# thanard/me-trpo

Hardware: AMD Instinct MI355X
Metric: imagined env-steps/sec (KxBxH) over the full TRPO iteration (higher is better)
Workload: dtype f32

## Files before the change

### me-trpo_amd/csrc/policy_mfma.hip

```cpp
#include <type_traits>
#include "device_common.h"
#include "cg_device.h"

typedef float f32x4 __attribute__((ext_vector_type(4)));
typedef float f32x2 __attribute__((ext_vector_type(2)));
#define PKFMA(a, b, c) __builtin_elementwise_fma((a), (b), (c))
#define MFMA16(a, b, c) __builtin_amdgcn_mfma_f32_16x16x4f32((a), (b), (c), 0, 0, 0)
#define PART_EXTRA 3
#ifndef POL_SKIP
#define POL_SKIP 0
#endif
#ifndef POL_SPLIT_R
#define POL_SPLIT_R 13
#endif
#ifndef POL_SPLIT_R_FVP
#define POL_SPLIT_R_FVP 7
#endif
#ifndef NWAVES
#define NWAVES 8
#endif
constexpr int cdiv_(int a, int b) { return (a + b - 1) / b; }
static_assert(POL_SPLIT_R == 0 || (NWAVES == 8 && (POL_SPLIT_R & 1) == 1 && POL_SPLIT_R >= 3 && (POL_SPLIT_R_FVP & 1) == 1 && POL_SPLIT_R_FVP >= 3), "the uneven deal pairs wave w with wave w + 4");
#ifdef POL_TIMING
__device__ unsigned long long g_pol_phase[16][8];
#define PT_MARK(i) { if (MODE_ == OP_FVPC && blockIdx.x == 0 && lane == 0) g_pol_phase[wave][i] = __builtin_readcyclecounter(); }
extern "C" int32_t metrpo_debug_pol_phases(unsigned long long* out) { return hipMemcpyFromSymbol(out, HIP_SYMBOL(g_pol_phase), sizeof(unsigned long long) * 128) == hipSuccess ? 0 : -1; }
#else
#define PT_MARK(i)
#endif


__device__ __forceinline__ void wave_sync_lds() {
    __builtin_amdgcn_fence(__ATOMIC_SEQ_CST, "wavefront");
    __builtin_amdgcn_wave_barrier();
}
__device__ __forceinline__ float xsum_q(float v) {
    typedef unsigned u32x2_ __attribute__((ext_vector_type(2)));
    const u32x2_ a = __builtin_amdgcn_permlane16_swap(__float_as_uint(v), __float_as_uint(v), false, false);
    const float s = __uint_as_float(a[0]) + __uint_as_float(a[1]);
    const u32x2_ b = __builtin_amdgcn_permlane32_swap(__float_as_uint(s), __float_as_uint(s), false, false);
    return __uint_as_float(b[0]) + __uint_as_float(b[1]);
}
template <int CTRL> __device__ __forceinline__ float dpp_add(float v) {
    return v + __int_as_float(__builtin_amdgcn_update_dpp(0, __float_as_int(v), CTRL, 0xF, 0xF, true));
}
__device__ __forceinline__ float xsum_c(float v) {
    v = dpp_add<0xB1>(v); v = dpp_add<0x4E>(v); v = dpp_add<0x141>(v); v = dpp_add<0x140>(v);
    return v;
}


template <int NS, int NA, int PH>
struct PolImg {
    static constexpr int NS_KS = cdiv_(NS, 4), HB = cdiv_(PH, 16), KK = HB * 4;
    static constexpr int O_W0F = 0, O_W1F = O_W0F + NS_KS * 64 * HB, O_V0F = O_W1F + KK * 64 * HB, O_V1F = O_V0F + NS_KS * 64 * HB,
                         O_W2B = O_V1F + KK * 64 * HB, O_W1B = O_W2B + 4 * 64 * HB, O_W2F = O_W1B + KK * 64 * HB,
                         O_V2F = O_W2F + KK * 64, TOTAL = O_V2F + KK * 64;
};


template <int NS, int NA, int PH, int MODE_>
__device__ __forceinline__ void pol_body(const PolK& k, const float* __restrict__ theta, const float* __restrict__ v, float* __restrict__ partials) {
    using I = PolImg<NS, NA, PH>;
    constexpr bool CACHED = (MODE_ == OP_FVPC), VPG = (MODE_ == OP_VPG), PPOKL = (MODE_ == OP_PPOKL), PPO = (MODE_ == OP_PPO) || PPOKL;
    constexpr int MODE = CACHED ? OP_FVP : (VPG || PPO) ? OP_GRAD : MODE_;
    constexpr int NS_KS = I::NS_KS, NSI = cdiv_(NS, 16), HB = I::HB, KK = I::KK;
    constexpr int pW0 = 0, pb0 = NS * PH, pW1 = pb0 + PH, pb1 = pW1 + PH * PH, pW2 = pb1 + PH, pb2 = pW2 + PH * NA,
                  pLS = pb2 + NA, P = pLS + NA, ROW = P + PART_EXTRA;
    constexpr int TS = 20, TILE = 16 * TS;
    constexpr int WTL = (3 * HB + (NA <= 2 ? 0 : 1)) * TILE;
    extern __shared__ __attribute__((aligned(16))) float lds[];
    const int tid = threadIdx.x, lane = tid & 63, wave = __builtin_amdgcn_readfirstlane(tid >> 6);
    const int c = lane & 15, q = lane >> 4;
    if (MODE_ == OP_LOSSKL && k.skip != nullptr && k.skip[0] >= 0.0) return;
    float* IMG = lds;
    float* TL = lds + I::TOTAL + wave * WTL;
    PT_MARK(0)
    const long long ntiles = (k.N + 15) / 16;
    const f32x4* __restrict__ hc = (const f32x4*)k.hcache;
    const bool ols_const = !VPG && (MODE != OP_FVP) && k.ls_stride == 0 && k.old_ls != nullptr;
    struct TileIn {
        float xB[NS_KS]; float xTs[4][NSI]; float ols[4], omu[4], act[4], adv; f32x4 gmv; int vld, nrem; f32x4 h[2 * HB];
    };
    auto fetch = [&](long long tile_, TileIn& in) {
        const long long tile = (tile_ < ntiles) ? tile_ : ntiles - 1;
        const long long n0 = tile * 16;
        const int nrem = (int)((k.N - n0 < 16) ? k.N - n0 : 16);
        in.nrem = nrem;
        const int cl = (c < nrem) ? c : nrem - 1;
        const float* __restrict__ ob = k.obs + n0 * NS;
#pragma unroll
        for (int s = 0; s < NS_KS; ++s) { const int f = 4 * s + q; in.xB[s] = ob[cl * NS + ((f < NS) ? f : NS - 1)]; }
        if (MODE != OP_LOSSKL) {
#pragma unroll
            for (int s = 0; s < 4; ++s) {
                const int sl = 4 * q + s, slc = (sl < nrem) ? sl : nrem - 1;
#pragma unroll
                for (int ci = 0; ci < NSI; ++ci) { const int f = 16 * ci + c; in.xTs[s][ci] = ob[slc * NS + ((f < NS) ? f : NS - 1)]; }
            }
        }
        in.vld = (k.valid == nullptr) ? 1 : (int)k.valid[n0 + cl];
        if (MODE != OP_FVP) {
            const long long nl = n0 + cl;
            if (MODE == OP_GRAD && k.gm != nullptr) {
#pragma unroll
                for (int r = 0; r < 4; ++r) { const int d = 4 * q + r; in.gmv[r] = k.gm[nl * NA + ((d < NA) ? d : NA - 1)]; }
            } else {
#pragma unroll
                for (int r = 0; r < 4; ++r) {
                    const int d = 4 * q + r, dc = (d < NA) ? d : NA - 1;
                    if (VPG) { in.act[r] = k.act[nl * NA + dc]; continue; }
                    in.ols[r] = ols_const ? 0.f : k.old_ls[(size_t)nl * k.ls_stride + dc]; in.omu[r] = k.old_mean[nl * NA + dc]; in.act[r] = k.act[nl * NA + dc];
                }
                in.adv = k.adv[nl];
            }
        }
        if (CACHED) {
            const f32x4* __restrict__ hb_ = hc + tile * (2 * HB) * 64;
#pragma unroll
            for (int j = 0; j < 2 * HB; ++j) in.h[j] = hb_[j * 64 + lane];
        }
    };
    auto mask_tile = [&](TileIn& in) {
#pragma unroll
        for (int s = 0; s < NS_KS; ++s) if (4 * s + 3 >= NS && 4 * s + q >= NS) in.xB[s] = 0.f;
        if (in.nrem == 16) return;
        const bool inr = c < in.nrem;
#pragma unroll
        for (int s = 0; s < NS_KS; ++s) if (!inr) in.xB[s] = 0.f;
#pragma unroll
        for (int s = 0; s < 4; ++s)
#pragma unroll
            for (int ci = 0; ci < NSI; ++ci) if (4 * q + s >= in.nrem) in.xTs[s][ci] = 0.f;
        if (!inr) { in.vld = 0; in.adv = 0.f; }
#pragma unroll
        for (int r = 0; r < 4; ++r) if (!inr) { in.ols[r] = 0.f; in.omu[r] = 0.f; in.act[r] = 0.f; in.gmv[r] = 0.f; }
    };
    TileIn nxt;

#define FRAG2(off, row, cb) IMG[(off) + ((row) * 64 + lane) * HB + (cb)]
#define FRAG1(off, row) IMG[(off) + (row) * 64 + lane]
    f32x4 b0f[HB], b1f[HB], b2f;
#pragma unroll
    for (int cb = 0; cb < HB; ++cb)
#pragma unroll
        for (int r = 0; r < 4; ++r) { const int u = 16 * cb + 4 * q + r; b0f[cb][r] = (u < PH) ? theta[pb0 + u] : 0.f; b1f[cb][r] = (u < PH) ? theta[pb1 + u] : 0.f; }
#pragma unroll
    for (int r = 0; r < 4; ++r) b2f[r] = (4 * q + r < NA) ? theta[pb2 + 4 * q + r] : 0.f;
    float ls[4], inv_std[4];
#pragma unroll
    for (int r = 0; r < 4; ++r) { ls[r] = (4 * q + r < NA) ? fmaxf(theta[pLS + 4 * q + r], LOG_MIN_STD) : 0.f; inv_std[r] = expf(-ls[r]); }
    float fisher_w[4];
#pragma unroll
    for (int r = 0; r < 4; ++r) fisher_w[r] = 1.0f / (expf(2.f * ls[r]) + 0.5f * KL_EPS);
    float ols_c[4] = {0.f, 0.f, 0.f, 0.f}, eo_c[4] = {1.f, 1.f, 1.f, 1.f}, os2_c[4] = {1.f, 1.f, 1.f, 1.f};
    if (ols_const) {
#pragma unroll
        for (int r = 0; r < 4; ++r)
            if (4 * q + r < NA) { ols_c[r] = k.old_ls[4 * q + r]; eo_c[r] = expf(-ols_c[r]); os2_c[r] = expf(2.f * ols_c[r]); }
    }
    constexpr bool kl_open = PPOKL;
    const float kl_w = PPOKL ? k.kl_beta * k.inv_n : 0.f, kl_d = PPOKL ? (float)k.kl_delta : 0.f;
    f32x4 vb0f[HB], vb1f[HB], vb2f;
    if (MODE == OP_FVP) {
#pragma unroll
        for (int cb = 0; cb < HB; ++cb)
#pragma unroll
            for (int r = 0; r < 4; ++r) { const int u = 16 * cb + 4 * q + r; vb0f[cb][r] = (u < PH) ? v[pb0 + u] : 0.f; vb1f[cb][r] = (u < PH) ? v[pb1 + u] : 0.f; }
#pragma unroll
        for (int r = 0; r < 4; ++r) vb2f[r] = (4 * q + r < NA) ? v[pb2 + 4 * q + r] : 0.f;
    }
    constexpr bool L2V = (NA <= 2);
    constexpr int NAV = L2V ? NA : 1;
    float w2l[HB][4][NAV], v2l[HB][4][NAV], gw2l[HB][4][NAV], b2l[NAV], vb2l[NAV], fisher_d[NAV];
    if (L2V) {
#pragma unroll
        for (int cb = 0; cb < HB; ++cb)
#pragma unroll
            for (int r = 0; r < 4; ++r)
#pragma unroll
                for (int d = 0; d < NAV; ++d) {
                    const int u = 16 * cb + 4 * q + r;
                    w2l[cb][r][d] = (u < PH) ? theta[pW2 + u * NA + d] : 0.f;
                    v2l[cb][r][d] = (MODE == OP_FVP && u < PH) ? v[pW2 + u * NA + d] : 0.f;
                    gw2l[cb][r][d] = 0.f;
                }
#pragma unroll
        for (int d = 0; d < NAV; ++d) {
            b2l[d] = theta[pb2 + d]; vb2l[d] = (MODE == OP_FVP) ? v[pb2 + d] : 0.f;
            fisher_d[d] = 1.0f / (expf(2.f * fmaxf(theta[pLS + d], LOG_MIN_STD)) + 0.5f * KL_EPS);
        }
    }
    constexpr int SPL = POL_SPLIT_R ? ((MODE == OP_GRAD || MODE_ == OP_FVP) ? POL_SPLIT_R : POL_SPLIT_R_FVP) : 0;
    const long long first_tile = SPL ? (long long)blockIdx.x * 4 + (wave & 3) + ((wave < 4) ? 0 : 1) * (long long)gridDim.x * 4 : (long long)blockIdx.x * NWAVES + wave;
    if (CACHED && k.imgval != nullptr) {
        static_assert(I::TOTAL % 4 == 0, "image tables are multiples of 64 floats");
        constexpr int NQ = I::TOTAL / 4, NIT = cdiv_(NQ, NWAVES * 64);
        float4 w4[NIT];
#pragma unroll
        for (int it = 0; it < NIT; ++it) { const int i = it * NWAVES * 64 + tid; w4[it] = (i < NQ) ? ((const float4*)k.imgval)[i] : make_float4(0.f, 0.f, 0.f, 0.f); }
        asm volatile("" ::: "memory");
        fetch(first_tile, nxt);
#pragma unroll
        for (int it = 0; it < NIT; ++it) { const int i = it * NWAVES * 64 + tid; if (i < NQ) ((float4*)IMG)[i] = w4[it]; }
    } else {
        constexpr int IMG_U = 8;
#pragma unroll
        for (int i0 = 0; i0 < I::TOTAL; i0 += NWAVES * 64 * IMG_U) {
            int m[IMG_U]; float w[IMG_U];
#pragma unroll
            for (int u = 0; u < IMG_U; ++u) { const int i = i0 + u * NWAVES * 64 + tid; m[u] = (i < I::TOTAL) ? k.img_map[i] : -1; }
#pragma unroll
            for (int u = 0; u < IMG_U; ++u) {
                const int i = i0 + u * NWAVES * 64 + tid;
                bool use = m[u] >= 0;
                if (MODE != OP_FVP && (m[u] & 0x40000000)) use = false;
                if (MODE == OP_LOSSKL && i >= I::O_W2B && i < I::O_W2F) use = false;
                if (CACHED && i < I::O_W1F) use = false;
                w[u] = 0.f;
                if (use) w[u] = (m[u] & 0x40000000) ? v[m[u] & 0x3FFFFFFF] : theta[m[u]];
            }
            if (i0 + NWAVES * 64 * IMG_U >= I::TOTAL) { asm volatile("" ::: "memory"); fetch(first_tile, nxt); asm volatile("" ::: "memory"); }
#pragma unroll
            for (int u = 0; u < IMG_U; ++u) { const int i = i0 + u * NWAVES * 64 + tid; if (i < I::TOTAL) IMG[i] = w[u]; }
        }
    }
    __syncthreads();
    if (MODE_ == OP_GRAD && k.imgval != nullptr && blockIdx.x == 0) {
        for (int i = tid; i < I::TOTAL; i += NWAVES * 64) k.imgval[i] = IMG[i];
    }
    PT_MARK(1)

    const f32x4 Z4 = {0.f, 0.f, 0.f, 0.f};
    f32x4 gW0[NSI][HB], gW1[HB][HB], gW2[HB], gb0[HB], gb1[HB], gb2 = Z4;
#pragma unroll
    for (int a = 0; a < HB; ++a) {
        gW2[a] = Z4; gb0[a] = Z4; gb1[a] = Z4;
#pragma unroll
        for (int b = 0; b < HB; ++b) gW1[a][b] = Z4;
#pragma unroll
        for (int b = 0; b < NSI; ++b) gW0[b][a] = Z4;
    }
    float dls[4] = {0.f, 0.f, 0.f, 0.f};
    float acc0 = 0.f, acc1 = 0.f, accw = 0.f;

    __builtin_amdgcn_s_waitcnt(0x0F70);
    PT_MARK(2)
    const long long sp_base = SPL ? (long long)blockIdx.x * 4 + (wave & 3) : (long long)blockIdx.x * NWAVES + wave, sp_stride = (long long)gridDim.x * (SPL ? 4 : NWAVES);
    auto sp_next = [&](long long m) -> long long {
        if constexpr (SPL == 0) return m + 1;
        else { const int ph = (int)(m % SPL); return (wave < 4) ? ((ph == SPL - 1) ? m + 1 : m + 2) : ((ph == SPL - 2) ? m + 3 : m + 2); }
    };
    for (long long m = (SPL && wave >= 4) ? 1 : 0, tile = sp_base + m * sp_stride; tile < ntiles; m = sp_next(m), tile = sp_base + m * sp_stride) {
        const long long n0 = tile * 16, n = n0 + c;
        const bool inr = n < k.N;
        TileIn in = nxt;
        fetch(sp_base + sp_next(m) * sp_stride, nxt);
        asm volatile("" ::: "memory");
        mask_tile(in);
        const bool ok = inr && in.vld != 0;
        const float (&xB)[NS_KS] = in.xB;
        const float (&xTs)[4][NSI] = in.xTs;
        const int wpos = c;
        float* T_H0 = TL, *T_H1 = TL + HB * TILE, *T_D1 = TL + 2 * HB * TILE, *T_UM = TL + 3 * HB * TILE;
        f32x4 h0[HB], h1[HB], t0[HB], t1[HB];
        constexpr bool H0C = CACHED;
        if (CACHED) {
#pragma unroll
            for (int cb = 0; cb < HB; ++cb) { if (H0C) h0[cb] = in.h[cb]; h1[cb] = in.h[HB + cb]; }
        }
#pragma unroll
        for (int cb = 0; cb < HB; ++cb) { if (!H0C) h0[cb] = b0f[cb]; if (MODE == OP_FVP) t0[cb] = vb0f[cb]; }
#pragma unroll
        for (int s = 0; s < NS_KS; ++s)
#pragma unroll
            for (int cb = 0; cb < HB; ++cb) {
                if (!H0C) h0[cb] = MFMA16(FRAG2(I::O_W0F, s, cb), xB[s], h0[cb]);
                if (MODE == OP_FVP) t0[cb] = MFMA16(FRAG2(I::O_V0F, s, cb), xB[s], t0[cb]);
            }
#pragma unroll
        for (int cb = 0; cb < HB; ++cb) {
            if (!CACHED) h1[cb] = b1f[cb];
            if (MODE == OP_FVP) t1[cb] = vb1f[cb];
            if (!H0C) {
#pragma unroll
                for (int r = 0; r < 4; ++r) h0[cb][r] = tanh_fast(h0[cb][r]);
            }
        }
#pragma unroll
        for (int kk = 0; kk < KK; ++kk)
#pragma unroll
            for (int cb = 0; cb < HB; ++cb) {
                if (!CACHED) h1[cb] = MFMA16(FRAG2(I::O_W1F, kk, cb), h0[kk >> 2][kk & 3], h1[cb]);
                if (MODE == OP_FVP) { if (POL_SKIP & 4) t1[cb][0] += h0[kk >> 2][kk & 3]; else t1[cb] = MFMA16(FRAG2(I::O_V1F, kk, cb), h0[kk >> 2][kk & 3], t1[cb]); }
            }
        if (MODE != OP_LOSSKL) {
#pragma unroll
            for (int cb = 0; cb < HB; ++cb)
#pragma unroll
                for (int r = 0; r < ((POL_SKIP & 8) ? 0 : 4); ++r) T_H0[cb * TILE + (4 * q + r) * TS + wpos] = h0[cb][r];
        }
        if (MODE == OP_FVP) {
#pragma unroll
            for (int cb = 0; cb < HB; ++cb)
#pragma unroll
                for (int r = 0; r < 4; ++r) t0[cb][r] *= fmaf(-h0[cb][r], h0[cb][r], 1.f);
#pragma unroll
            for (int kk = 0; kk < KK; ++kk)
#pragma unroll
                for (int cb = 0; cb < HB; ++cb) { if (POL_SKIP & 4) t1[cb][1] += t0[kk >> 2][kk & 3]; else t1[cb] = MFMA16(FRAG2(I::O_W1F, kk, cb), t0[kk >> 2][kk & 3], t1[cb]); }
        }
        if (!CACHED) {
#pragma unroll
            for (int cb = 0; cb < HB; ++cb)
#pragma unroll
                for (int r = 0; r < 4; ++r) h1[cb][r] = tanh_fast(h1[cb][r]);
        }
        if (MODE != OP_LOSSKL) {
#pragma unroll
            for (int cb = 0; cb < HB; ++cb)
#pragma unroll
                for (int r = 0; r < (((POL_SKIP & 8) || NA <= 2) ? 0 : 4); ++r) T_H1[cb * TILE + (4 * q + r) * TS + wpos] = h1[cb][r];
        }
        if (MODE == OP_GRAD && k.hcache != nullptr) {
            f32x4* hw = (f32x4*)k.hcache + (size_t)tile * (2 * HB) * 64 + lane;
#pragma unroll
            for (int cb = 0; cb < HB; ++cb) { hw[cb * 64] = h0[cb]; hw[(HB + cb) * 64] = h1[cb]; }
        }

        f32x4 um = Z4;
        float ual[NAV];
#pragma unroll
        for (int d = 0; d < NAV; ++d) ual[d] = 0.f;
        if (MODE == OP_GRAD && k.gm != nullptr) {
#pragma unroll
            for (int r = 0; r < 4; ++r) um[r] = (ok && 4 * q + r < NA) ? in.gmv[r] : 0.f;
        } else if (MODE != OP_FVP) {
            f32x4 mu = Z4;
            if (L2V) {
#pragma unroll
                for (int d = 0; d < NAV; ++d) {
                    float a = 0.f;
#pragma unroll
                    for (int cb = 0; cb < HB; ++cb)
#pragma unroll
                        for (int r = 0; r < 4; ++r) a = fmaf(w2l[cb][r][d], h1[cb][r], a);
                    a = xsum_q(a) + b2l[d];
                    if (q == 0) mu[d] = a;
                }
            } else {
                f32x4 m0 = b2f, m1 = Z4;
#pragma unroll
                for (int kk = 0; kk < KK; kk += 2) {
                    m0 = MFMA16(FRAG1(I::O_W2F, kk), h1[kk >> 2][kk & 3], m0);
                    m1 = MFMA16(FRAG1(I::O_W2F, kk + 1), h1[(kk + 1) >> 2][(kk + 1) & 3], m1);
                }
                mu = m0 + m1;
            }
            float llr = 0.f, kl = 0.f, zz[4] = {0.f, 0.f, 0.f, 0.f};
            float kmu[4] = {0.f, 0.f, 0.f, 0.f}, kls[4] = {0.f, 0.f, 0.f, 0.f};
#pragma unroll
            for (int r = 0; r < 4; ++r) {
                const int d = 4 * q + r;
                if (VPG && d < NA && ok) {
                    const float z = (in.act[r] - mu[r]) * inv_std[r];
                    llr -= ls[r] + 0.5f * z * z;
                    zz[r] = z;
                } else if (d < NA && ok) {
                    const float omu = in.omu[r], a = in.act[r];
                    float ols, eo, os2 = 0.f;
                    if (ols_const) { ols = ols_c[r]; eo = eo_c[r]; os2 = os2_c[r]; }
                    else {
                        ols = in.ols[r];
                        asm volatile("" : "+v"(ols));
                        eo = expf(-ols);
                        if (MODE == OP_LOSSKL || (PPOKL && kl_open)) os2 = expf(2.f * ols);
                    }
                    const float z = (a - mu[r]) * inv_std[r], zo = (a - omu) * eo;
                    llr += (ols - ls[r]) + 0.5f * (zo * zo - z * z);
                    zz[r] = z;
                    if (MODE == OP_LOSSKL) {
                        const float s2 = expf(2.f * ls[r]), dm = omu - mu[r];
                        kl += (dm * dm + os2 - s2) / (2.f * s2 + KL_EPS) + ls[r] - ols;
                    }
                    if constexpr (PPOKL) { if (kl_open) kl += ppo_kl_dim(mu[r], omu, ls[r], ols, os2, inv_std[r], &kmu[r], &kls[r]); }
                }
            }
            llr = xsum_q(llr);
            float la, surr;
            if constexpr (PPO) { la = ppo_gate(expf(llr), in.adv, k.clip_lo, k.clip_hi, &surr); if (!ok) { la = 0.f; surr = 0.f; } }
            else { la = ok ? (VPG ? in.adv : expf(llr) * in.adv) : 0.f; surr = VPG ? (llr - NA * HALF_LOG_2PI) * la : la; }
            if (q == 0) acc0 -= surr * k.inv_n;
            if (MODE == OP_LOSSKL) { acc1 += kl * k.inv_n; continue; }
            const float w = -la * k.inv_n;
#pragma unroll
            for (int r = 0; r < 4; ++r) {
                um[r] = w * zz[r] * inv_std[r];
                if (4 * q + r < NA) dls[r] += w * (zz[r] * zz[r] - 1.f);
            }
            if constexpr (PPOKL) {
                if (kl_open) {
                    acc0 += kl_w * kl;
                    if (q == 0 && ok) acc0 -= kl_w * kl_d;
#pragma unroll
                    for (int r = 0; r < 4; ++r) { um[r] += kl_w * kmu[r]; if (4 * q + r < NA) dls[r] += kl_w * kls[r]; }
                }
            }
        } else {
            f32x4 m0 = vb2f, m1 = Z4;
            if (!L2V) {
#pragma unroll
                for (int kk = 0; kk < KK; ++kk) m1 = MFMA16(FRAG1(I::O_V2F, kk), h1[kk >> 2][kk & 3], m1);
            }
#pragma unroll
            for (int cb = 0; cb < HB; ++cb)
#pragma unroll
                for (int r = 0; r < 4; ++r) t1[cb][r] *= fmaf(-h1[cb][r], h1[cb][r], 1.f);
            if (L2V) {
                m0 = Z4;
                float av[NAV];
                if constexpr (NAV == 2) {
                    f32x2 a2 = {0.f, 0.f};
#pragma unroll
                    for (int cb = 0; cb < HB; ++cb)
#pragma unroll
                        for (int r = 0; r < 4; ++r)
                            a2 = PKFMA((f32x2{w2l[cb][r][0], w2l[cb][r][1]}), (f32x2{t1[cb][r], t1[cb][r]}),
                                       PKFMA((f32x2{v2l[cb][r][0], v2l[cb][r][1]}), (f32x2{h1[cb][r], h1[cb][r]}), a2));
                    av[0] = a2[0]; av[1] = a2[1];
                } else {
#pragma unroll
                    for (int d = 0; d < NAV; ++d) {
                        av[d] = 0.f;
#pragma unroll
                        for (int cb = 0; cb < HB; ++cb)
#pragma unroll
                            for (int r = 0; r < 4; ++r) av[d] = fmaf(w2l[cb][r][d], t1[cb][r], fmaf(v2l[cb][r][d], h1[cb][r], av[d]));
                    }
                }
#pragma unroll
                for (int d = 0; d < NAV; ++d) {
                    const float a = xsum_q(av[d]) + vb2l[d];
                    if (q == 0) m0[d] = a;
                    ual[d] = ok ? a * fisher_d[d] * k.inv_n : 0.f;
                }
            } else {
#pragma unroll
                for (int kk = 0; kk < KK; ++kk) m0 = MFMA16(FRAG1(I::O_W2F, kk), t1[kk >> 2][kk & 3], m0);
            }
#pragma unroll
            for (int r = 0; r < 4; ++r)
                um[r] = (ok && 4 * q + r < NA) ? (m0[r] + m1[r]) * fisher_w[r] * k.inv_n : 0.f;
            if (ok && q == 0) accw += k.inv_n;
        }
        f32x4 d1[HB], d0n[HB];
#pragma unroll
        for (int cb = 0; cb < HB; ++cb) d1[cb] = Z4;
        if (L2V) {
            float ua[NAV];
#pragma unroll
            for (int d = 0; d < NAV; ++d) ua[d] = (MODE == OP_FVP) ? ual[d] : __shfl(um[d], c, 64);
#pragma unroll
            for (int cb = 0; cb < HB; ++cb)
#pragma unroll
                for (int r = 0; r < 4; ++r) {
#pragma unroll
                    for (int d = 0; d < NAV; ++d) d1[cb][r] = fmaf(w2l[cb][r][d], ua[d], d1[cb][r]);
                    if constexpr (NAV == 2) {
                        const f32x2 g2 = PKFMA((f32x2{h1[cb][r], h1[cb][r]}), (f32x2{ua[0], ua[1]}), (f32x2{gw2l[cb][r][0], gw2l[cb][r][1]}));
                        gw2l[cb][r][0] = g2[0]; gw2l[cb][r][1] = g2[1];
                    } else {
#pragma unroll
                        for (int d = 0; d < NAV; ++d) gw2l[cb][r][d] = fmaf(h1[cb][r], ua[d], gw2l[cb][r][d]);
                    }
                }
        } else {
#pragma unroll
            for (int r = 0; r < 4; ++r) T_UM[(4 * q + r) * TS + wpos] = um[r];
#pragma unroll
            for (int r = 0; r < 4; ++r) {
                if (r >= NA) continue;
#pragma unroll
                for (int cb = 0; cb < HB; ++cb) d1[cb] = MFMA16(FRAG2(I::O_W2B, r, cb), um[r], d1[cb]);
            }
        }
#pragma unroll
        for (int cb = 0; cb < HB; ++cb) {
            d0n[cb] = Z4;
#pragma unroll
            for (int r = 0; r < 4; ++r) { d1[cb][r] *= fmaf(-h1[cb][r], h1[cb][r], 1.f); T_D1[cb * TILE + (4 * q + r) * TS + wpos] = d1[cb][r]; }
        }
#pragma unroll
        for (int kk = 0; kk < KK; ++kk)
#pragma unroll
            for (int cb = 0; cb < HB; ++cb) { if (POL_SKIP & 4) d0n[cb][2] += d1[kk >> 2][kk & 3]; else d0n[cb] = MFMA16(d1[kk >> 2][kk & 3], FRAG2(I::O_W1B, kk, cb), d0n[cb]); }
        gb2 += um;
#pragma unroll
        for (int cb = 0; cb < HB; ++cb) gb1[cb] += d1[cb];
        wave_sync_lds();
        f32x4 a1v[HB], a0v[HB], b1v[HB], buv = Z4;
#pragma unroll
        for (int cb = 0; cb < HB; ++cb) {
            a1v[cb] = *(const f32x4*)&T_H1[cb * TILE + c * TS + 4 * q]; a0v[cb] = *(const f32x4*)&T_H0[cb * TILE + c * TS + 4 * q];
            b1v[cb] = *(const f32x4*)&T_D1[cb * TILE + c * TS + 4 * q];
        }
#pragma unroll
        for (int cb = 0; cb < HB; ++cb) {
#pragma unroll
            for (int r = 0; r < 4; ++r) d0n[cb][r] *= fmaf(-a0v[cb][r], a0v[cb][r], 1.f);
            gb0[cb] += d0n[cb];
        }
        if (!L2V) buv = *(const f32x4*)&T_UM[c * TS + 4 * q];
#pragma unroll
        for (int s = 0; s < ((POL_SKIP & 2) ? 0 : 4); ++s) {
            const float bu = buv[s];
            float a1_[HB], a0_[HB], b1_[HB], b0_[HB], xT[NSI];
#pragma unroll
            for (int cb = 0; cb < HB; ++cb) { a1_[cb] = a1v[cb][s]; a0_[cb] = a0v[cb][s]; b1_[cb] = b1v[cb][s]; b0_[cb] = d0n[cb][s]; }
#pragma unroll
            for (int ci = 0; ci < NSI; ++ci) xT[ci] = xTs[s][ci];
            if (POL_SKIP & 1) { gW1[0][0][0] += a0_[0] + b1_[0] + a1_[0] + b0_[0] + xT[0] + a0_[HB - 1] + b1_[HB - 1] + a1_[HB - 1] + b0_[HB - 1] + bu; continue; }
            if (!L2V) {
#pragma unroll
                for (int ci = 0; ci < HB; ++ci) gW2[ci] = MFMA16(a1_[ci], bu, gW2[ci]);
            }
#pragma unroll
            for (int ci = 0; ci < HB; ++ci)
#pragma unroll
                for (int cj = 0; cj < HB; ++cj) gW1[ci][cj] = MFMA16(a0_[ci], b1_[cj], gW1[ci][cj]);
#pragma unroll
            for (int ci = 0; ci < NSI; ++ci)
#pragma unroll
                for (int cj = 0; cj < HB; ++cj) gW0[ci][cj] = MFMA16(xT[ci], b0_[cj], gW0[ci][cj]);
        }
        wave_sync_lds();
    }
#undef FRAG2
#undef FRAG1

    PT_MARK(3)
    __syncthreads();
    PT_MARK(4)
    float* RB = lds;
    float* row = RB + wave * ROW;
    if (MODE != OP_GRAD && lane < NA) row[pLS + lane] = 0.f;
    wave_sync_lds();
    if (MODE != OP_LOSSKL) {
#pragma unroll
        for (int r = 0; r < 4; ++r) {
#pragma unroll
            for (int cj = 0; cj < HB; ++cj) {
                const int j = 16 * cj + c;
#pragma unroll
                for (int ci = 0; ci < NSI; ++ci) { const int i = 16 * ci + 4 * q + r; if (i < NS && j < PH) row[pW0 + i * PH + j] = gW0[ci][cj][r]; }
#pragma unroll
                for (int ci = 0; ci < HB; ++ci) { const int i = 16 * ci + 4 * q + r; if (i < PH && j < PH) row[pW1 + i * PH + j] = gW1[ci][cj][r]; }
            }
            if (L2V) {
#pragma unroll
                for (int ci = 0; ci < HB; ++ci)
#pragma unroll
                    for (int d = 0; d < NAV; ++d) {
                        const float sg = xsum_c(gw2l[ci][r][d]);
                        const int i = 16 * ci + 4 * q + r;
                        if (c == 0 && i < PH) row[pW2 + i * NA + d] = sg;
                    }
            } else {
#pragma unroll
                for (int ci = 0; ci < HB; ++ci) { const int i = 16 * ci + 4 * q + r; if (i < PH && c < NA) row[pW2 + i * NA + c] = gW2[ci][r]; }
            }
#pragma unroll
            for (int cb = 0; cb < HB; ++cb) {
                const float s1 = xsum_c(gb1[cb][r]);
                const int u = 16 * cb + 4 * q + r;
                if (c == 0 && u < PH) row[pb1 + u] = s1;
            }
            if (r == 0) {
#pragma unroll
                for (int cb = 0; cb < HB; ++cb) {
                    const float s0 = xsum_q((gb0[cb][0] + gb0[cb][1]) + (gb0[cb][2] + gb0[cb][3]));
                    if (q == 0 && 16 * cb + c < PH) row[pb0 + 16 * cb + c] = s0;
                }
            }
            const float s2 = xsum_c(gb2[r]), sl = xsum_c(dls[r]);
            if (c == 0 && 4 * q + r < NA) {
                row[pb2 + 4 * q + r] = s2;
                if (MODE == OP_GRAD) row[pLS + 4 * q + r] = (theta[pLS + 4 * q + r] > LOG_MIN_STD) ? sl : 0.f;
            }
        }
    }
    if (PPO) {
        acc1 = 0.f;
        if (blockIdx.x == 0 && wave == 0 && c == 0) {
            acc1 = (q == 0) ? NA * ENTROPY_CONST : 0.f;
#pragma unroll
            for (int r = 0; r < 4; ++r) if (4 * q + r < NA) acc1 += ls[r];
        }
    }
    {
        const float a0 = xsum_c(xsum_q(acc0)), a1 = xsum_c(xsum_q(acc1)), aw = xsum_c(xsum_q(accw));
        if (lane == 0) { row[P] = a0; row[P + 1] = a1; row[P + 2] = aw; }
    }
    __syncthreads();
    PT_MARK(5)
    float* out = partials + (size_t)blockIdx.x * ROW;
    for (int i = (MODE == OP_LOSSKL ? P : 0) + tid; i < ROW; i += NWAVES * 64) {
        float a = 0.f;
#pragma unroll
        for (int w = 0; w < NWAVES; w += 4) a += (RB[w * ROW + i] + RB[(w + 1) * ROW + i]) + (RB[(w + 2) * ROW + i] + RB[(w + 3) * ROW + i]);
        out[i] = a;
    }
    PT_MARK(6)
}

template <int NS, int NA, int PH, int MODE_>
__global__ void __launch_bounds__(NWAVES * 64, 1) k_policy_mfma(PolK k, const float* __restrict__ theta, const float* __restrict__ v,
                                                        float* __restrict__ partials) {
    if constexpr (MODE_ == OP_PPOKL) {
        if (!ppo_kl_open(k.mean_kl, k.kl_delta)) { pol_body<NS, NA, PH, OP_PPO>(k, theta, v, partials); return; }
    }
    pol_body<NS, NA, PH, MODE_>(k, theta, v, partials);
}


template <int NS, int NA, int PH>
static void pol_image_map(std::vector<int>& map) {
    using I = PolImg<NS, NA, PH>;
    constexpr int HB = I::HB;
    constexpr int pW0 = 0, pb0 = NS * PH, pW1 = pb0 + PH, pb1 = pW1 + PH * PH, pW2 = pb1 + PH;
    const int VFLAG = 0x40000000;
    map.assign(I::TOTAL, -1);
    for (int i = 0; i < I::TOTAL; ++i) {
        int m = -1;
        if (i < I::O_W2F) {
            int t, base;
            if (i < I::O_W1F) { t = 0; base = I::O_W0F; } else if (i < I::O_V0F) { t = 1; base = I::O_W1F; }
            else if (i < I::O_V1F) { t = 2; base = I::O_V0F; } else if (i < I::O_W2B) { t = 3; base = I::O_V1F; }
            else if (i < I::O_W1B) { t = 4; base = I::O_W2B; } else { t = 5; base = I::O_W1B; }
            const int j = i - base, cb = j % HB, ln = (j / HB) & 63, row = j / (HB * 64), cc = ln & 15, qq = ln >> 4;
            const int flag = (t == 2 || t == 3) ? VFLAG : 0;
            if (t == 0 || t == 2) { const int in = 4 * row + qq, o = 16 * cb + cc; if (in < NS && o < PH) m = (pW0 + in * PH + o) | flag; }
            else if (t == 1 || t == 3) { const int in = 16 * (row >> 2) + 4 * qq + (row & 3), o = 16 * cb + cc; if (in < PH && o < PH) m = (pW1 + in * PH + o) | flag; }
            else if (t == 4) { const int ii = 16 * cb + cc, d = 4 * qq + row; if (ii < PH && d < NA) m = pW2 + ii * NA + d; }
            else { const int ii = 16 * cb + cc, jj = 16 * (row >> 2) + 4 * qq + (row & 3); if (ii < PH && jj < PH) m = pW1 + ii * PH + jj; }
        } else {
            const bool isv = i >= I::O_V2F;
            const int j = i - (isv ? I::O_V2F : I::O_W2F), ln = j & 63, row = j >> 6, cc = ln & 15, qq = ln >> 4;
            const int in = 16 * (row >> 2) + 4 * qq + (row & 3);
            if (in < PH && cc < NA) m = (pW2 + in * NA + cc) | (isv ? VFLAG : 0);
        }
        map[i] = m;
    }
}

typedef void (*pol_kernel_t)(PolK, const float*, const float*, float*);
struct PolEntry { int ns, na, ph; pol_kernel_t kern[7] ; int lds_floats, lds_floats_eval; void (*build_map)(std::vector<int>&); };
template <int NS, int NA, int PH> constexpr int pol_lds() {
    constexpr int HB = cdiv_(PH, 16);
    constexpr int a = PolImg<NS, NA, PH>::TOTAL + NWAVES * (3 * HB + (NA <= 2 ? 0 : 1)) * 16 * 20;
    constexpr int P = NS * PH + PH + PH * PH + PH + PH * NA + NA + NA;
    constexpr int b = NWAVES * (P + PART_EXTRA);
    return a > b ? a : b;
}
template <int NS, int NA, int PH> constexpr int pol_lds_eval() {
    constexpr int P = NS * PH + PH + PH * PH + PH + PH * NA + NA + NA;
    constexpr int a = PolImg<NS, NA, PH>::TOTAL, b = NWAVES * (P + PART_EXTRA);
    return a > b ? a : b;
}
#define PENTRY(NS, NA, PH) {NS, NA, PH, {k_policy_mfma<NS, NA, PH, OP_GRAD>, k_policy_mfma<NS, NA, PH, OP_FVP>, k_policy_mfma<NS, NA, PH, OP_LOSSKL>, k_policy_mfma<NS, NA, PH, OP_FVPC>, k_policy_mfma<NS, NA, PH, OP_VPG>, k_policy_mfma<NS, NA, PH, OP_PPO>, k_policy_mfma<NS, NA, PH, OP_PPOKL>}, pol_lds<NS, NA, PH>(), pol_lds_eval<NS, NA, PH>(), pol_image_map<NS, NA, PH>}
static const PolEntry kPol[] = {
    PENTRY(10, 2, 32),
    PENTRY(18, 6, 32),
    PENTRY(11, 3, 32),
    PENTRY(14, 4, 32),
    PENTRY(29, 8, 32),
};

int policy_mfma_select(const ProblemDesc& pd) {
    if (pd.pol.n_layers != 3 || pd.pol.dims[1] != pd.pol.dims[2]) return -1;
    for (int i = 0; i < (int)(sizeof(kPol) / sizeof(kPol[0])); ++i)
        if (kPol[i].ns == pd.ns && kPol[i].na == pd.na && kPol[i].ph == pd.pol.dims[1]) return i;
    return -1;
}

int policy_mfma_image_buffers(metrpo_ctx* c) {
    const int idx = c->pol_mfma;
    if (idx < 0) return set_err(c, METRPO_EUNSUPPORTED, "no MFMA policy kernels for this shape");
    if (c->pol_img_idx == idx) return METRPO_OK;
    const PolEntry& en = kPol[idx];
    std::vector<int> map;
    en.build_map(map);
    std::vector<int> vpos((size_t)c->pd.P, -1);
    for (size_t i = 0; i < map.size(); ++i)
        if (map[i] >= 0 && (map[i] & 0x40000000)) {
            const int j = map[i] & 0x3FFFFFFF;
            if (j >= c->pd.P || vpos[j] != -1) return set_err(c, METRPO_EINVAL, "policy image map: tangent entry out of range or stored twice");
            vpos[j] = (int)i;
        }
    c->pol_img_idx = -1;
    int rc;
    if ((rc = ws_grow(c, c->d_pol_img, sizeof(int) * map.size())) || (rc = ws_grow(c, c->d_pol_vpos, sizeof(int) * vpos.size())) ||
        (rc = ws_grow(c, c->d_pol_imgval, sizeof(float) * map.size())))
        return rc;
    HIP_TRY(c, hipMemcpy(c->d_pol_img.p, map.data(), sizeof(int) * map.size(), hipMemcpyHostToDevice));
    HIP_TRY(c, hipMemcpy(c->d_pol_vpos.p, vpos.data(), sizeof(int) * vpos.size(), hipMemcpyHostToDevice));
    HIP_TRY(c, hipMemset(c->d_pol_imgval.p, 0, sizeof(float) * map.size()));
    c->pol_img_idx = idx;
    return METRPO_OK;
}

int policy_mfma_launch(metrpo_ctx* c, const UpdCall& u, float* partials, int nblocks, hipStream_t st) {
    const PolEntry& en = kPol[c->pol_mfma];
    { const int rc = policy_mfma_image_buffers(c); if (rc) return rc; }
    PolK k = u.k;
    int mode = u.op;
    k.img_map = (const int*)c->d_pol_img.p;
    k.hcache = nullptr;
    const bool cached = u.scope.cache_activations && (mode == OP_GRAD || mode == OP_FVP) && k.gm == nullptr;
    k.imgval = (u.scope.publish_image && cached) ? c->d_pol_imgval.p : nullptr;
    if (cached) {
        const size_t need = (size_t)((k.N + 15) / 16) * 2 * (size_t)cdiv_(en.ph, 16) * 64 * 4;
        { const int rc = ws_grow(c, c->d_hcache, need * sizeof(float)); if (rc) return rc; }
        k.hcache = c->d_hcache.p;
        if (mode == OP_FVP) mode = OP_FVPC;
    }
    size_t sh = sizeof(float) * (size_t)en.lds_floats;
    if (mode == OP_LOSSKL) sh = sizeof(float) * (size_t)en.lds_floats_eval;
    if (sh > 64 * 1024) HIP_TRY(c, hipFuncSetAttribute((const void*)en.kern[mode], hipFuncAttributeMaxDynamicSharedMemorySize, (int)sh));
    hipLaunchKernelGGL(en.kern[mode], dim3(nblocks), dim3(NWAVES * 64), sh, st, k, u.theta, u.vf, partials);
    HIP_TRY(c, hipGetLastError());
    return METRPO_OK;
}
```

Measured before the change: 1.968 billion.

## Specialize policy kernel on mean-adjoint and double-buffer tile prefetch loop

Adds a compile-time VJP template flag so the gradient kernel branches once at launch on whether a mean adjoint is supplied, instead of testing it per tile. The tile loop becomes a do_tile lambda driven by two alternating TileIn buffers, which removes the per-iteration struct copy. The loop also tracks the split phase incrementally in place of a modulo, and the valid-flag load is made branchless. Several compiler-steering asm barriers, per-NA loop trimming and address-space casts are added to shape register allocation and codegen, at the cost of extra template instantiations and more fragile code.

Measured after the change: 2.000 billion (median of 6 runs). +1.6%, better.

```diff
diff --git a/me-trpo_amd/csrc/policy_mfma.hip b/me-trpo_amd/csrc/policy_mfma.hip
--- a/me-trpo_amd/csrc/policy_mfma.hip
+++ b/me-trpo_amd/csrc/policy_mfma.hip
@@ -59,11 +59,14 @@
 };
 
 
-template <int NS, int NA, int PH, int MODE_>
+__device__ const uint8_t g_pol_valid_one = 1;
+
+template <int NS, int NA, int PH, int MODE_, bool VJP>
 __device__ __forceinline__ void pol_body(const PolK& k, const float* __restrict__ theta, const float* __restrict__ v, float* __restrict__ partials) {
     using I = PolImg<NS, NA, PH>;
     constexpr bool CACHED = (MODE_ == OP_FVPC), VPG = (MODE_ == OP_VPG), PPOKL = (MODE_ == OP_PPOKL), PPO = (MODE_ == OP_PPO) || PPOKL;
     constexpr int MODE = CACHED ? OP_FVP : (VPG || PPO) ? OP_GRAD : MODE_;
+    static_assert(!VJP || MODE_ == OP_GRAD, "the mean-adjoint is an input of the plain gradient kernel only");
     constexpr int NS_KS = I::NS_KS, NSI = cdiv_(NS, 16), HB = I::HB, KK = I::KK;
     constexpr int pW0 = 0, pb0 = NS * PH, pW1 = pb0 + PH, pb1 = pW1 + PH * PH, pW2 = pb1 + PH, pb2 = pW2 + PH * NA,
                   pLS = pb2 + NA, P = pLS + NA, ROW = P + PART_EXTRA;
@@ -78,11 +81,15 @@
     PT_MARK(0)
     const long long ntiles = (k.N + 15) / 16;
     const f32x4* __restrict__ hc = (const f32x4*)k.hcache;
-    const bool ols_const = !VPG && (MODE != OP_FVP) && k.ls_stride == 0 && k.old_ls != nullptr;
+    const bool ols_const = !VPG && !VJP && (MODE != OP_FVP) && k.ls_stride == 0 && k.old_ls != nullptr;
     struct TileIn {
         float xB[NS_KS]; float xTs[4][NSI]; float ols[4], omu[4], act[4], adv; f32x4 gmv; int vld, nrem; f32x4 h[2 * HB];
     };
-    auto fetch = [&](long long tile_, TileIn& in) {
+    constexpr int NR = (NA < 4) ? NA : 4;
+    typedef const uint8_t __attribute__((address_space(1)))* gu8_p;
+    const gu8_p vld_p = (gu8_p)((k.valid != nullptr) ? k.valid : &g_pol_valid_one);
+    const int vld_m = (k.valid != nullptr) ? -1 : 0;
+    auto fetch = [&](long long tile_, TileIn& in) __attribute__((always_inline)) {
         const long long tile = (tile_ < ntiles) ? tile_ : ntiles - 1;
         const long long n0 = tile * 16;
         const int nrem = (int)((k.N - n0 < 16) ? k.N - n0 : 16);
@@ -99,18 +106,18 @@
                 for (int ci = 0; ci < NSI; ++ci) { const int f = 16 * ci + c; in.xTs[s][ci] = ob[slc * NS + ((f < NS) ? f : NS - 1)]; }
             }
         }
-        in.vld = (k.valid == nullptr) ? 1 : (int)k.valid[n0 + cl];
+        in.vld = (int)(vld_p + (n0 & (long long)vld_m))[cl & vld_m];
         if (MODE != OP_FVP) {
             const long long nl = n0 + cl;
-            if (MODE == OP_GRAD && k.gm != nullptr) {
-#pragma unroll
-                for (int r = 0; r < 4; ++r) { const int d = 4 * q + r; in.gmv[r] = k.gm[nl * NA + ((d < NA) ? d : NA - 1)]; }
+            if constexpr (VJP) {
+#pragma unroll
+                for (int r = 0; r < NR; ++r) { const int d = 4 * q + r; in.gmv[r] = k.gm[nl * NA + ((d < NA) ? d : NA - 1)]; }
             } else {
 #pragma unroll
-                for (int r = 0; r < 4; ++r) {
+                for (int r = 0; r < NR; ++r) {
                     const int d = 4 * q + r, dc = (d < NA) ? d : NA - 1;
                     if (VPG) { in.act[r] = k.act[nl * NA + dc]; continue; }
-                    in.ols[r] = ols_const ? 0.f : k.old_ls[(size_t)nl * k.ls_stride + dc]; in.omu[r] = k.old_mean[nl * NA + dc]; in.act[r] = k.act[nl * NA + dc];
+                    in.ols[r] = k.old_ls[(size_t)nl * k.ls_stride + dc]; in.omu[r] = k.old_mean[nl * NA + dc]; in.act[r] = k.act[nl * NA + dc];
                 }
                 in.adv = k.adv[nl];
             }
@@ -121,20 +128,21 @@
             for (int j = 0; j < 2 * HB; ++j) in.h[j] = hb_[j * 64 + lane];
         }
     };
-    auto mask_tile = [&](TileIn& in) {
+    auto mask_tile = [&](TileIn& in) __attribute__((always_inline)) {
 #pragma unroll
         for (int s = 0; s < NS_KS; ++s) if (4 * s + 3 >= NS && 4 * s + q >= NS) in.xB[s] = 0.f;
         if (in.nrem == 16) return;
         const bool inr = c < in.nrem;
 #pragma unroll
         for (int s = 0; s < NS_KS; ++s) if (!inr) in.xB[s] = 0.f;
+        if (!inr) in.vld = 0;
 #pragma unroll
         for (int s = 0; s < 4; ++s)
 #pragma unroll
             for (int ci = 0; ci < NSI; ++ci) if (4 * q + s >= in.nrem) in.xTs[s][ci] = 0.f;
-        if (!inr) { in.vld = 0; in.adv = 0.f; }
-#pragma unroll
-        for (int r = 0; r < 4; ++r) if (!inr) { in.ols[r] = 0.f; in.omu[r] = 0.f; in.act[r] = 0.f; in.gmv[r] = 0.f; }
+        if (!inr) in.adv = 0.f;
+#pragma unroll
+        for (int r = 0; r < NR; ++r) if (!inr) { in.ols[r] = 0.f; in.omu[r] = 0.f; in.act[r] = 0.f; in.gmv[r] = 0.f; }
     };
     TileIn nxt;
 
@@ -247,15 +255,19 @@
     __builtin_amdgcn_s_waitcnt(0x0F70);
     PT_MARK(2)
     const long long sp_base = SPL ? (long long)blockIdx.x * 4 + (wave & 3) : (long long)blockIdx.x * NWAVES + wave, sp_stride = (long long)gridDim.x * (SPL ? 4 : NWAVES);
-    auto sp_next = [&](long long m) -> long long {
-        if constexpr (SPL == 0) return m + 1;
-        else { const int ph = (int)(m % SPL); return (wave < 4) ? ((ph == SPL - 1) ? m + 1 : m + 2) : ((ph == SPL - 2) ? m + 3 : m + 2); }
+    const int ph_last = (wave < 4) ? SPL - 1 : SPL - 2, ph_first = (wave < 4) ? 0 : 1, m_wrap = (wave < 4) ? 1 : 3;
+    auto sp_next = [&](long long& m, int& ph) __attribute__((always_inline)) {
+        if constexpr (SPL == 0) m += 1;
+        else { const bool last = (ph == ph_last); m += last ? m_wrap : 2; ph = last ? ph_first : ph + 2; }
     };
-    for (long long m = (SPL && wave >= 4) ? 1 : 0, tile = sp_base + m * sp_stride; tile < ntiles; m = sp_next(m), tile = sp_base + m * sp_stride) {
+    constexpr bool HEAD_ARM = (NA == 3) || (NA == 2 && (MODE_ == OP_GRAD || MODE_ == OP_PPO)) || PPOKL;
+    constexpr int SQ_PIN = ((NA == 4 || NA == 8) && (MODE_ == OP_GRAD || MODE_ == OP_PPO)) ? 0 : -1;
+    int head_off = 0;
+    asm volatile("" : "+s"(head_off));
+    auto do_tile = [&](const long long tile, TileIn& in, const long long tile_pre, TileIn& pre) __attribute__((always_inline)) {
         const long long n0 = tile * 16, n = n0 + c;
         const bool inr = n < k.N;
-        TileIn in = nxt;
-        fetch(sp_base + sp_next(m) * sp_stride, nxt);
+        fetch(tile_pre, pre);
         asm volatile("" ::: "memory");
         mask_tile(in);
         const bool ok = inr && in.vld != 0;
@@ -332,9 +344,12 @@
         float ual[NAV];
 #pragma unroll
         for (int d = 0; d < NAV; ++d) ual[d] = 0.f;
-        if (MODE == OP_GRAD && k.gm != nullptr) {
-#pragma unroll
-            for (int r = 0; r < 4; ++r) um[r] = (ok && 4 * q + r < NA) ? in.gmv[r] : 0.f;
+        if constexpr (VJP) {
+#pragma unroll
+            for (int r = 0; r < NR; ++r) um[r] = (ok && 4 * q + r < NA) ? in.gmv[r] : 0.f;
+        } else if (MODE == OP_GRAD && HEAD_ARM && head_off) {
+#pragma unroll
+            for (int r = 0; r < NR; ++r) um[r] = (ok && 4 * q + r < NA) ? in.act[r] : 0.f;
         } else if (MODE != OP_FVP) {
             f32x4 mu = Z4;
             if (L2V) {
@@ -360,7 +375,7 @@
             float llr = 0.f, kl = 0.f, zz[4] = {0.f, 0.f, 0.f, 0.f};
             float kmu[4] = {0.f, 0.f, 0.f, 0.f}, kls[4] = {0.f, 0.f, 0.f, 0.f};
 #pragma unroll
-            for (int r = 0; r < 4; ++r) {
+            for (int r = 0; r < NR; ++r) {
                 const int d = 4 * q + r;
                 if (VPG && d < NA && ok) {
                     const float z = (in.act[r] - mu[r]) * inv_std[r];
@@ -391,12 +406,19 @@
             if constexpr (PPO) { la = ppo_gate(expf(llr), in.adv, k.clip_lo, k.clip_hi, &surr); if (!ok) { la = 0.f; surr = 0.f; } }
             else { la = ok ? (VPG ? in.adv : expf(llr) * in.adv) : 0.f; surr = VPG ? (llr - NA * HALF_LOG_2PI) * la : la; }
             if (q == 0) acc0 -= surr * k.inv_n;
-            if (MODE == OP_LOSSKL) { acc1 += kl * k.inv_n; continue; }
+            if (MODE == OP_LOSSKL) { acc1 += kl * k.inv_n; return; }
             const float w = -la * k.inv_n;
 #pragma unroll
             for (int r = 0; r < 4; ++r) {
                 um[r] = w * zz[r] * inv_std[r];
-                if (4 * q + r < NA) dls[r] += w * (zz[r] * zz[r] - 1.f);
+                if constexpr (SQ_PIN < 0) {
+                    if (4 * q + r < NA) dls[r] += w * (zz[r] * zz[r] - 1.f);
+                } else {
+                    float zm1;
+                    if (r == SQ_PIN) { float sq = zz[r] * zz[r]; asm volatile("" : "+v"(sq)); zm1 = sq - 1.f; }
+                    else zm1 = __builtin_fmaf(zz[r], zz[r], -1.f);
+                    if (4 * q + r < NA) dls[r] += w * zm1;
+                }
             }
             if constexpr (PPOKL) {
                 if (kl_open) {
@@ -405,6 +427,10 @@
 #pragma unroll
                     for (int r = 0; r < 4; ++r) { um[r] += kl_w * kmu[r]; if (4 * q + r < NA) dls[r] += kl_w * kls[r]; }
                 }
+            }
+            if constexpr (!HEAD_ARM) {
+#pragma unroll
+                for (int r = 0; r < 4; ++r) { float x = um[r]; asm volatile("" : "+v"(x)); um[r] = x; }
             }
         } else {
             f32x4 m0 = vb2f, m1 = Z4;
@@ -534,6 +560,28 @@
                 for (int cj = 0; cj < HB; ++cj) gW0[ci][cj] = MFMA16(xT[ci], b0_[cj], gW0[ci][cj]);
         }
         wave_sync_lds();
+    };
+    {
+        constexpr bool TWO_BUF = !(VPG || PPOKL);
+        TileIn nxt2;
+        long long m = (SPL && wave >= 4) ? 1 : 0;
+        int ph = (int)m;
+        long long tile = sp_base + m * sp_stride;
+        while (tile < ntiles) {
+            sp_next(m, ph);
+            const long long tile1 = sp_base + m * sp_stride;
+            if constexpr (TWO_BUF) {
+                do_tile(tile, nxt, tile1, nxt2);
+                if (!(tile1 < ntiles)) break;
+                sp_next(m, ph);
+                tile = sp_base + m * sp_stride;
+                do_tile(tile1, nxt2, tile, nxt);
+            } else {
+                TileIn cur = nxt;
+                do_tile(tile, cur, tile1, nxt);
+                tile = tile1;
+            }
+        }
     }
 #undef FRAG2
 #undef FRAG1
@@ -541,6 +589,9 @@
     PT_MARK(3)
     __syncthreads();
     PT_MARK(4)
+    typedef const float __attribute__((address_space(1)))* gf32_p;
+    gf32_p th_e = (gf32_p)theta;
+    asm volatile("" : "+s"(th_e));
     float* RB = lds;
     float* row = RB + wave * ROW;
     if (MODE != OP_GRAD && lane < NA) row[pLS + lane] = 0.f;
@@ -585,7 +636,7 @@
             const float s2 = xsum_c(gb2[r]), sl = xsum_c(dls[r]);
             if (c == 0 && 4 * q + r < NA) {
                 row[pb2 + 4 * q + r] = s2;
-                if (MODE == OP_GRAD) row[pLS + 4 * q + r] = (theta[pLS + 4 * q + r] > LOG_MIN_STD) ? sl : 0.f;
+                if (MODE == OP_GRAD) row[pLS + 4 * q + r] = (th_e[pLS + 4 * q + r] > LOG_MIN_STD) ? sl : 0.f;
             }
         }
     }
@@ -594,7 +645,7 @@
         if (blockIdx.x == 0 && wave == 0 && c == 0) {
             acc1 = (q == 0) ? NA * ENTROPY_CONST : 0.f;
 #pragma unroll
-            for (int r = 0; r < 4; ++r) if (4 * q + r < NA) acc1 += ls[r];
+            for (int r = 0; r < 4; ++r) if (4 * q + r < NA) acc1 += fmaxf(th_e[pLS + 4 * q + r], LOG_MIN_STD);
         }
     }
     {
@@ -617,9 +668,17 @@
 __global__ void __launch_bounds__(NWAVES * 64, 1) k_policy_mfma(PolK k, const float* __restrict__ theta, const float* __restrict__ v,
                                                         float* __restrict__ partials) {
     if constexpr (MODE_ == OP_PPOKL) {
-        if (!ppo_kl_open(k.mean_kl, k.kl_delta)) { pol_body<NS, NA, PH, OP_PPO>(k, theta, v, partials); return; }
-    }
-    pol_body<NS, NA, PH, MODE_>(k, theta, v, partials);
+        if (!ppo_kl_open(k.mean_kl, k.kl_delta)) {
+            typedef const float __attribute__((address_space(1)))* gf32_p;
+            gf32_p th = (gf32_p)theta;
+            asm volatile("" : "+s"(th));
+            pol_body<NS, NA, PH, OP_PPO, false>(k, (const float*)th, v, partials); return;
+        }
+    }
+    if constexpr (MODE_ == OP_GRAD) {
+        if (k.gm != nullptr) { pol_body<NS, NA, PH, OP_GRAD, true>(k, theta, v, partials); return; }
+    }
+    pol_body<NS, NA, PH, MODE_, false>(k, theta, v, partials);
 }
 
 
```
